# jianzongwu/betrayed-by-captions

Measured on AMD Instinct MI355X. Metric: images/sec (COCO-shaped 1024x1024, 100 queries, forward-only), higher is better.
Workload: dtype f32; 1 GPU; configs[1]: R50 + 100 queries, 1024x1024, batch 2/GPU, forward-only; global_batch=2, parallelism=replicas x1, precision=fp32 (parity mode, f16x3 MFMA), hip_graph=True, x3_overflow=False, library_fallbacks=0

## Files before the change

betrayed-by-captions_amd/_lib.py:

```python
import ctypes
import os

import torch

_HERE = os.path.dirname(os.path.abspath(__file__))
LIB_PATH = os.path.join(_HERE, 'lib', 'libcgg_hip.so')

CGG_F32 = 0
CGG_BF16 = 1

_c_int = ctypes.c_int
_c_vp = ctypes.c_void_p
_c_f = ctypes.c_float
_c_i64 = ctypes.c_int64

PROTOTYPES = {
    'cgg_version': (_c_int, []),
    'cgg_init': (_c_int, [_c_int]),
    'cgg_msda_forward_fused_vld': (_c_int, [_c_vp, _c_int, _c_vp, _c_vp, _c_vp, _c_int, _c_vp, _c_vp] + [_c_int] * 7 + [_c_vp]),
    'cgg_msda_backward_hostlevels_ws': (_c_int, [_c_vp, _c_int] + [_c_vp] * 8 + [_c_int] * 8 + [_c_vp, _c_i64, _c_vp, _c_vp]),
    'cgg_msda_backward_workspace_bytes': (_c_i64, [_c_vp, _c_vp] + [_c_int] * 7),
    'cgg_msda_read_levels': (_c_int, [_c_vp, _c_vp, _c_int, _c_int, _c_vp, _c_vp, _c_vp]),
    'cgg_last_error_string': (ctypes.c_char_p, []),
    'cgg_msda_forward': (_c_int, [_c_vp] * 6 + [_c_int] * 8 + [_c_vp]),
# ... 61 lines not shown
                       [_c_int] * 4 + [_c_vp]),
    'cgg_conv_x3_nhwc': (_c_int, [_c_vp] * 5 + [_c_int] * 10 + [_c_vp]),
    'cgg_gemm_x3s': (_c_int, [_c_vp, _c_int, _c_vp, _c_vp, _c_vp, _c_int, _c_int, _c_int, _c_vp, _c_int, _c_int] + [_c_int] * 4 + [_c_vp]),
    'cgg_gemm_x3s_batched': (_c_int, [_c_vp, _c_int, _c_int, _c_i64, _c_vp, _c_vp, _c_vp, _c_int, _c_int, _c_int, _c_vp, _c_int, _c_int] + [_c_int] * 4 + [_c_vp]),
    'cgg_conv_x3s_nhwc': (_c_int, [_c_vp] * 4 + [_c_int, _c_vp, _c_int] + [_c_int] * 10 + [_c_vp]),
    'cgg_x3a_encode': (_c_int, [_c_vp, _c_vp, _c_i64, _c_vp]),
    'cgg_x3a_decode': (_c_int, [_c_vp, _c_vp, _c_i64, _c_vp]),
    'cgg_x3_overflow_check': (_c_int, [_c_int, _c_vp, _c_vp]),
    'cgg_gemm_x3s_cfg': (_c_int, [_c_vp, _c_int, _c_vp, _c_vp, _c_vp, _c_int, _c_int, _c_int, _c_vp, _c_int, _c_int] + [_c_int] * 5 + [_c_vp]),
    'cgg_conv_x3s_nhwc_cfg': (_c_int, [_c_vp] * 4 + [_c_int, _c_vp, _c_int] + [_c_int] * 11 + [_c_vp]),
    'cgg_bias_relu_maxpool_nhwc_f32_x3a': (_c_int, [_c_vp] * 3 + [_c_int] * 4 + [_c_vp]),
    'cgg_group_norm_nhwc_f32_x3a': (_c_int, [_c_vp] * 4 + [_c_int] * 4 + [_c_f, _c_int, _c_vp, _c_int, _c_int, _c_i64, _c_int, _c_vp,
                                             _c_i64, _c_vp, _c_vp, _c_vp]),
    'cgg_encoder_layer_tail_x3a': (_c_int, [_c_vp] * 6 + [_c_f] + [_c_vp] * 6 + [_c_f, _c_vp, _c_int, _c_vp, _c_vp] +
                                   [_c_int] * 3 + [_c_vp]),
    'cgg_wgrad_x3_workspace_bytes': (_c_i64, [_c_int] * 3),
    'cgg_wgrad_x3': (_c_int, [_c_vp, _c_int, _c_vp, _c_int, _c_vp, _c_vp] + [_c_int] * 3 + [_c_vp]),
    'cgg_wgrad_bias_x3': (_c_int, [_c_vp, _c_int, _c_vp, _c_int, _c_vp, _c_vp, _c_vp] + [_c_int] * 3 + [_c_vp]),
    'cgg_transpose_f32': (_c_int, [_c_vp, _c_vp, _c_int, _c_int, _c_int, _c_vp]),
    'cgg_nchw_to_nhwc_pad1_f32': (_c_int, [_c_vp, _c_vp] + [_c_int] * 4 + [_c_vp]),
    'cgg_topk_select': (_c_int, [_c_vp, _c_int, _c_int, _c_int, _c_int, _c_vp, _c_vp]),
    'cgg_absmax_f32': (_c_int, [_c_vp, _c_int, _c_int, _c_int, _c_vp, _c_vp]),
    'cgg_relu_bwd_absmax_f32': (_c_int, [_c_vp, _c_vp, _c_vp, ctypes.c_longlong, _c_vp, _c_vp]),
    'cgg_gemm_x3_bwd': (_c_int, [_c_vp, _c_int, _c_vp, _c_vp, _c_vp, _c_int, _c_vp, _c_int, _c_vp] + [_c_int] * 3 + [_c_vp]),
    'cgg_gemm_x3_scaled': (_c_int, [_c_vp, _c_int, _c_vp, _c_vp, _c_vp, _c_vp, _c_int, _c_vp, _c_int] + [_c_int] * 4 + [_c_vp]),
    'cgg_conv_x3_nhwc_scaled': (_c_int, [_c_vp] * 6 + [_c_int] * 10 + [_c_vp]),
    'cgg_wgrad_x3_scaled': (_c_int, [_c_vp, _c_int, _c_vp, _c_vp, _c_int, _c_vp, _c_vp, _c_vp] + [_c_int] * 3 + [_c_vp]),
    'cgg_layernorm_chain': (_c_int, [_c_vp, _c_int, _c_vp, _c_vp, _c_f, _c_vp, _c_int, _c_vp, _c_vp, _c_f, _c_vp, _c_vp,
                                     _c_vp, _c_int, _c_int, _c_int, _c_i64, _c_vp]),
    'cgg_msda_prologue': (_c_int, [_c_vp, _c_int, _c_vp, _c_vp, _c_vp, _c_vp] + [_c_int] * 5 + [_c_vp]),
# ... 115 lines not shown
```

betrayed-by-captions_amd/csrc/norm.hip:

```cpp
#include "x3.h"

#define GN_CHUNK 16384

template <int VEC>
__global__ __launch_bounds__(256) void cgg_gn_partial_kernel(const float* __restrict__ x,
                                                             float* __restrict__ part, long long row_len,
                                                             int chunks) {
  const int row = blockIdx.y, chunk = blockIdx.x;
  const long long beg = (long long)chunk * GN_CHUNK;
  const long long end = min(row_len, beg + GN_CHUNK);
  const float* xr = x + (size_t)row * row_len;
  float s = 0.f, ss = 0.f;
  if (VEC == 4) {
    for (long long i = beg + threadIdx.x * 4; i < end; i += 256 * 4) {
      const f32x4 v = *reinterpret_cast<const f32x4*>(xr + i);
      s += (v[0] + v[1]) + (v[2] + v[3]);
      ss += (v[0] * v[0] + v[1] * v[1]) + (v[2] * v[2] + v[3] * v[3]);
    }
  } else {
    for (long long i = beg + threadIdx.x; i < end; i += 256) {
      const float v = xr[i];
      s += v;
      ss += v * v;
    }
// ... 366 lines not shown
                                              int W, float* y_padded, cgg_stream_t stream) {
  CGG_REQUIRE(y_padded && W > 0 && HW % W == 0, CGG_EINVAL, "cgg_group_norm_nhwc_f32_padout: null output / bad W");
  return gnh_launch(true, x, gamma, beta, ws, B, HW, C, groups, eps, relu, up_src, up_h, up_w, up_bstride, W, y_padded,
                    (int64_t)(HW / W + 2) * (W + 2) * C, nullptr, nullptr, nullptr, 0, stream, nullptr, 0, W);
}

extern "C" int cgg_group_norm_nhwc_f32_x3a(const float* x, const float* gamma, const float* beta, void* ws, int B, int HW, int C,
                                           int groups, float eps, int relu, const void* up_src_x3a, int up_h, int up_w,
                                           int64_t up_bstride, int W, void* y_x3a, int64_t y_bstride, const float* pos,
                                           void* yp_x3a, cgg_stream_t stream) {
  CGG_REQUIRE(y_x3a, CGG_EINVAL, "cgg_group_norm_nhwc_f32_x3a: null output");
  return gnh_launch(true, x, gamma, beta, ws, B, HW, C, groups, eps, relu, (const float*)up_src_x3a, up_h, up_w, up_bstride, W,
                    (float*)y_x3a, y_bstride, nullptr, pos, nullptr, 0, stream, (float*)yp_x3a, up_src_x3a ? 3 : 1);
}

template <bool RELU>
__global__ __launch_bounds__(256) void cgg_gn_nhwc_bwd_partials_kernel(const float* __restrict__ x, const float* __restrict__ y,
                                                                      const float* __restrict__ dy, const float* __restrict__ stats,
                                                                      float eps, float* __restrict__ part, int HW, int G, int ppb) {
  __shared__ float red[16][256];
  const int b = blockIdx.y, tid = threadIdx.x;
  const int g = tid % G, pl = tid / G, PL = 256 / G;
  const int p0 = blockIdx.x * ppb, p1 = min(p0 + ppb, HW);
  const float mean = stats[((size_t)b * G + g) * 2], rstd = rsqrtf(stats[((size_t)b * G + g) * 2 + 1] + eps);
  float dg[8], db[8];
#pragma unroll
  for (int k = 0; k < 8; ++k) dg[k] = db[k] = 0.f;
  for (int p = p0 + pl; p < p1; p += PL) {
    const size_t o = (((size_t)b * HW + p) * G + g) * 8;
    const f32x4 xa = *reinterpret_cast<const f32x4*>(x + o), xb = *reinterpret_cast<const f32x4*>(x + o + 4);
// ... 183 lines not shown
```

betrayed-by-captions_amd/mask2former_head.py:

```python
import copy
import os
import json
import warnings

import torch
import torch.distributed as dist
import torch.nn as nn
import torch.nn.functional as F

from . import ops, runtime
from .assigner import get_uncertain_point_coords_with_randomness, point_sample
from .bert_embeddings import BertEmbeddings
from .config import ConfigDict, to_config_dict
from .registry import (HEADS, build_assigner, build_head, build_loss, build_plugin_layer,
                       build_positional_encoding, build_sampler, build_transformer_layer_sequence)

POINT_LOGITS_X3 = os.environ.get('CGG_POINT_LOGITS_X3', '1') != '0'
BOS_TOKEN = 101
EOS_TOKEN = 102


def get_dist_info():
    if dist.is_available() and dist.is_initialized():
        return dist.get_rank(), dist.get_world_size()
# ... 486 lines not shown

    @staticmethod
    def _pack_stream(mf, sizes):
        H4, W4 = int(mf.shape[1]), int(mf.shape[2])
        pools = []
        for (h, w) in sizes:
            s = H4 // h
            pools.append(s if (h * s == H4 and w * s == W4 and s in (2, 4, 8)) else None)
        uniq = [1] + sorted({p for p in pools if p is not None})
        if len(uniq) <= 4:
            packed = dict(zip(uniq, ops.pack_mask_feature_nhwc_multi(mf, uniq)))
        else:
            packed = {p: ops.pack_mask_feature_nhwc(mf, p) for p in uniq}
        return packed[1], [packed[p] if p is not None else None for p in pools]

    def _finish_encode(self, enc):
        if enc.get('x3a'):
            sizes, memorys = enc['sizes'], enc['memorys']
            mf = enc['mf'] if 'mf' in enc else self.pixel_decoder.stream_fpn_x3a(*enc['fpn'])
            H4, W4 = int(mf.shape[1]), int(mf.shape[2])
            pools = []
            for h, w in sizes:
                s = H4 // h
                pools.append(s if (h * s == H4 and w * s == W4 and s in (2, 4, 8)) else None)
            uniq = [1] + sorted({p for p in pools if p is not None})
            packed = dict(zip(uniq, ops.pack_mask_feature_nhwc_x3(mf, uniq)))
            return dict(stream=True, kvs=self._project_kv_x3a(memorys, sizes), sizes=sizes, packed_full=packed[1],
                        pooled=[packed[p] if p is not None else None for p in pools], mask_features=None)
        kv16, sizes = enc['kv16'], enc['sizes']
        mf = enc['mf'] if 'mf' in enc else self.pixel_decoder.stream_fpn(*enc['fpn'])
        L = self.num_transformer_feat_level
        layers = self.transformer_decoder.layers
        H4, W4 = int(mf.shape[1]), int(mf.shape[2])
        packed_full, pooled = self._pack_stream(mf, sizes)
        kvs = self._project_kv_levels(kv16)
        return dict(stream=True, kvs=kvs, sizes=sizes, packed_full=packed_full, pooled=pooled, mask_features=None)

    def _project_kv_levels(self, kv16):
        L = self.num_transformer_feat_level
        layers = self.transformer_decoder.layers
        nl = self.num_transformer_decoder_layers
# ... 62 lines not shown
                return dict(stream=True, deferred=True, mf=mf, kv16=kv16, sizes=[level_hw[i] for i in range(L)])
            for i in range(L):
                sizes.append(level_hw[i])
                if kv16 is None:
                    mems.append(memorys[i] + self.level_embed.weight[i].view(1, 1, -1))
                    poss.append(self.decoder_positional_encoding.flat_unpadded(level_hw[i][0], level_hw[i][1], mf.device))
            packed_full, pooled = self._pack_stream(mf, sizes)
        elif (hasattr(pd, 'stream_ready_x3') and pd.stream_ready_x3(feats) and pd.num_outs >= L
              and all(isinstance(p, nn.Identity) for p in self.decoder_input_projs)
              and self.transformer_decoder.post_norm is not None and self.query_embed.weight.shape[1] % 32 == 0
              and all(l.stream_ready() for l in self.transformer_decoder.layers)):
            if defer_tail and runtime.x3a_enabled():
                mf, memorys, level_hw = pd.forward_stream_x3(feats, defer_fpn=defer_tail == 2)
                return dict(stream=True, deferred=True, x3a=True, memorys=memorys, sizes=[level_hw[i] for i in range(L)],
                            **({'fpn': mf} if defer_tail == 2 else {'mf': mf}))
            mf, memorys, level_hw = pd.forward_stream_x3(feats)
            mask_features = None
            H4, W4 = int(mf.shape[1]), int(mf.shape[2])
            pools = []
            x3a_mem = all(ops.is_x3a(m) for m in memorys[:L])
            for i in range(L):
                h, w = level_hw[i]
                sizes.append((h, w))
                if not x3a_mem:
                    mems.append(memorys[i] + self.level_embed.weight[i].view(1, 1, -1))
                    poss.append(self.decoder_positional_encoding.flat_unpadded(h, w, mf.device))
                s = H4 // h
                pools.append(s if (h * s == H4 and w * s == W4 and s in (2, 4, 8)) else None)
            uniq = [1] + sorted({p for p in pools if p is not None})
            packed = dict(zip(uniq, ops.pack_mask_feature_nhwc_x3(mf, uniq)))
            packed_full, pooled = packed[1], [packed[p] if p is not None else None for p in pools]
            if x3a_mem:
                kvs = self._project_kv_x3a(memorys, sizes)
                return dict(stream=True, kvs=kvs, sizes=sizes, packed_full=packed_full, pooled=pooled, mask_features=None)
        else:
            if runtime.x3_enabled() and not torch.is_grad_enabled() and feats[0].is_cuda:
                runtime.note_fallback('pixel decoder / head', 'stream_ready_x3() is false for this configuration: module path on f32 '
                                      'library GEMMs')
            feats = [ops.x3a_to_f32(f) if ops.is_x3a(f) else f for f in feats]
            feats = [f.float().contiguous() if f.dtype != torch.float32 else f for f in feats]
            mask_features, memorys = pd(feats)
            mask_features = mask_features.contiguous()
            split = not runtime.is_bf16()
            H4, W4 = mask_features.shape[-2:]
            for i in range(L):
# ... 711 lines not shown
```

betrayed-by-captions_amd/ops.py:

```python
import ctypes
import os
import math

import torch

from . import _lib
from ._lib import CGG_BF16, CGG_F32, CggError, check, dev_ptr, stream_ptr

_WS_CACHE = {}

KERNEL_EVENTS = None


KERNEL_META = None


class _timed:
    def __init__(self, name, **meta):
        self.name = name
        self.meta = meta
        self.on = KERNEL_EVENTS is not None and not torch.cuda.is_current_stream_capturing()

    def __enter__(self):
        if self.on:
# ... 1130 lines not shown
    if x.dtype != torch.float32:
        raise CggError(f'group_norm_nhwc_x3a: x dtype {x.dtype}')
    need = _lib_().cgg_group_norm_nhwc_workspace_bytes(B, HW, int(groups))
    if ws is None or ws.numel() * ws.element_size() < need:
        raise CggError(f'group_norm_nhwc_x3a: workspace too small ({need} bytes needed; see group_norm_nhwc_workspace)')
    rc = _lib_().cgg_group_norm_nhwc_f32_x3a(
        dev_ptr(x, 'x', torch.float32), dev_ptr(gamma, 'gamma', torch.float32), dev_ptr(beta, 'beta', torch.float32),
        dev_ptr(ws, 'ws', torch.float32), B, HW, C, int(groups), float(eps), int(bool(relu)),
        _ptr_at(up[0], up[1]) if up is not None else None, up[3] if up is not None else 0,
        up[4] if up is not None else 0, up[2] if up is not None else 0, int(W),
        _ptr_at(out[0], out[1]), out[2], _ptr_at(pos[0], pos[1]) if pos is not None else None,
        _ptr_at(outp[0], outp[1]) if outp is not None else None, stream_ptr(x.device))
    check(rc, 'cgg_group_norm_nhwc_f32_x3a')


def zero_border_map(B, H, W, C, device):
    y = torch.empty((B, H + 2, W + 2, C), dtype=torch.float32, device=device)
    y[:, 0].zero_()
    y[:, H + 1].zero_()
    y[:, 1:H + 1, 0].zero_()
    y[:, 1:H + 1, W + 1].zero_()
    return y


def group_norm_nhwc_padout(x, gamma, beta, groups, eps, ws, hw, y_padded, relu=False, lo=None, lo_hw=None):
    B, HW, C = x.shape
    H, W = int(hw[0]), int(hw[1])
    if x.dtype != torch.float32 or not x.is_contiguous() or tuple(y_padded.shape) != (B, H + 2, W + 2, C) or not y_padded.is_contiguous():
        raise CggError('group_norm_nhwc_padout: x (B, HW, C) float32 contiguous and y_padded (B, H + 2, W + 2, C) expected')
    if lo is not None and (not lo.is_contiguous() or lo.dtype != torch.float32):
# ... 68 lines not shown
    for pool in pools:
        if H % pool or W % pool:
            raise CggError(f'pack_mask_feature_nhwc_x3: {H}x{W} not divisible by pool={pool}')
        h, w = H // pool, W // pool
        hi = torch.empty((B, (h * w + 31) // 32, C // 8, 32, 8), dtype=torch.bfloat16, device=feat.device)
        lo = torch.empty_like(hi)
        outs.append(PackedFeature(hi, lo, B, C, h, w))
        hp.append(hi.data_ptr())
        lp.append(lo.data_ptr())
    n = len(pools)
    rc = _lib_().cgg_pack_mask_feature_nhwc_f32_x3(dev_ptr(feat, 'mask_feature', torch.float32), (ctypes.c_void_p * n)(*hp),
                                                   (ctypes.c_void_p * n)(*lp), _int_array([int(p) for p in pools]), n,
                                                   B, C, H, W, stream_ptr(feat.device))
    check(rc, 'cgg_pack_mask_feature_nhwc_f32_x3')
    return outs


def pack_mask_feature_nhwc_multi(feat, pools):
    B, H, W, C = feat.shape
    outs, ptrs = [], []
    for pool in pools:
        if H % pool or W % pool:
            raise CggError(f'pack_mask_feature_nhwc: {H}x{W} not divisible by pool={pool}')
        h, w = H // pool, W // pool
        hi = torch.empty((B, (h * w + 31) // 32, C // 8, 32, 8), dtype=torch.bfloat16, device=feat.device)
        outs.append(PackedFeature(hi, None, B, C, h, w))
        ptrs.append(hi.data_ptr())
    n = len(pools)
    rc = _lib_().cgg_pack_mask_feature_nhwc_multi(dev_ptr(feat, 'mask_feature', torch.bfloat16),
                                                  (ctypes.c_void_p * n)(*ptrs), _int_array([int(p) for p in pools]), n,
# ... 905 lines not shown
```

betrayed-by-captions_amd/pixel_decoder.py:

```python
import math
import os

import torch
import torch.nn as nn
import torch.nn.functional as F

from . import ops, runtime
from .registry import (ATTENTION, FEEDFORWARD_NETWORK, PLUGIN_LAYERS, POSITIONAL_ENCODING,
                       TRANSFORMER_LAYER, TRANSFORMER_LAYER_SEQUENCE, build_attention,
                       build_feedforward_network, build_positional_encoding,
                       build_transformer_layer, build_transformer_layer_sequence)

FUSED_TAIL = os.environ.get('CGG_FUSED_TAIL', '1') != '0'
FUSED_TRAIN_MSDA = os.environ.get('CGG_FUSED_TRAIN_MSDA', '1') != '0'
FUSED_TRAIN_LN = os.environ.get('CGG_FUSED_TRAIN_LN', '1') != '0'
MERGED_PROJ = os.environ.get('CGG_MERGED_PROJ', '1') != '0' and not os.environ.get('CGG_MSDA_GENERIC')


def build_norm(cfg, num_features):
    cfg = dict(cfg)
    t = cfg.pop('type')
    requires_grad = cfg.pop('requires_grad', True)
    if t == 'GN':
        m = nn.GroupNorm(cfg.pop('num_groups'), num_features, **cfg)
# ... 792 lines not shown
        cache[key] = (ver, t)
        while len(cache) > 2 * len(self.encoder.layers):
            cache.popitem(last=False)
        return runtime.keepalive(t)

    @staticmethod
    def _merged_proj_ok(layer):
        attn = layer.attentions[0]
        so, aw, vp = attn.sampling_offsets, attn.attention_weights, attn.value_proj
        C, H = vp.weight.shape[1], attn.num_heads
        n_cat = so.weight.shape[0] + aw.weight.shape[0]
        return (MERGED_PROJ and H == 8 and C == 256 and vp.weight.shape[0] == 256 and attn.num_levels == 3 and attn.num_points == 4
                and n_cat == 3 * H * attn.num_levels * attn.num_points and (C + n_cat) % 32 == 0
                and all(m.bias is not None for m in (vp, so, aw)))

    def _forward_stream_x3a(self, feats, defer_fpn=False):
        B = feats[0].shape[0]
        dev = feats[0].device
        C = 256
        rows = lambda f: (f if ops.is_x3a(f) else ops.x3a_encode(ops.nchw_to_nhwc(f).contiguous()).permute(0, 3, 1, 2)) \
            .as_subclass(torch.Tensor).permute(0, 2, 3, 1).reshape(-1, f.shape[1])
        level_hw, level_start, N, pos, ref = self._stream_levels(feats)
        src = torch.empty((B, N, C), dtype=torch.float32, device=dev)
        need_srcp = not all(self._merged_proj_ok(l) for l in self.encoder.layers)
        srcp = torch.empty((B, N, C), dtype=torch.float32, device=dev) if need_srcp else None
        ws = ops.group_norm_nhwc_workspace(B, int(feats[0].shape[2]) * int(feats[0].shape[3]), 32, dev)
        for i in range(self.num_encoder_levels):
            f = feats[self.num_input_levels - i - 1]
            h, w = level_hw[i]
            cm = self.input_convs[i]
            y = runtime.linear_x3s(rows(f), cm.conv.weight.flatten(1), cm.conv.bias)
            gn = getattr(cm, cm.norm_name)
            ops.group_norm_nhwc_x3a(y.view(B, h * w, C), gn.weight, gn.bias, 32, gn.eps, ws, out=(src, level_start[i] * C, N * C),
                                    pos=(pos, level_start[i] * C) if need_srcp else None,
                                    outp=(srcp, level_start[i] * C) if need_srcp else None)
        src = self._encoder_stream_x3a(src, srcp, pos, ref, level_hw, level_start)
        mems = [ops.as_x3a(src[:, s0:s0 + h * w, :]) for s0, (h, w) in zip(level_start, level_hw)]
        fpn = (rows(feats[0]), int(feats[0].shape[2]), int(feats[0].shape[3]), src, level_start[-1], N, level_hw[-1], ws)
        if defer_fpn:
            return fpn, mems, level_hw
        return self.stream_fpn_x3a(*fpn), mems, level_hw

    def stream_fpn_x3a(self, frows, H4, W4, src, fine_start, N, fine_hw, ws):
        C = 256
        B = src.shape[0]
        lat, outc = self.lateral_convs[0], self.output_convs[0]
        hl, wl = fine_hw
        level_start = [fine_start]
        y = runtime.linear_x3s(frows, lat.conv.weight.flatten(1), lat.conv.bias).view(B, H4 * W4, C)
        gn = getattr(lat, lat.norm_name)
        ops.group_norm_nhwc_x3a(y, gn.weight, gn.bias, 32, gn.eps, ws, out=(y, 0, H4 * W4 * C),
                                up=(src, level_start[-1] * C, N * C, hl, wl), W=W4)
        w3 = runtime.derived_cached('x3_conv_image', (outc.conv.weight,), lambda: ops.pack_conv_weight_x3(outc.conv.weight))
        z = ops.conv_x3s_nhwc(y.view(B, H4, W4, C), w3, C, 3, 1, 1, outc.conv.bias, out_split=False).view(B, H4 * W4, C)
        gn = getattr(outc, outc.norm_name)
        ops.group_norm_nhwc_x3a(z, gn.weight, gn.bias, 32, gn.eps, ws, out=(z, 0, H4 * W4 * C), relu=True)
        mf = runtime.linear_x3s(z.view(B * H4 * W4, C), self.mask_feature.weight.flatten(1), self.mask_feature.bias)
        return mf.view(B, H4, W4, -1)

    def forward_stream_x3(self, feats, defer_fpn=False):
        if runtime.x3a_enabled():
            return self._forward_stream_x3a(feats, defer_fpn=defer_fpn)
        feats = [ops.x3a_to_f32(f) if ops.is_x3a(f) else f for f in feats]
        B = feats[0].shape[0]
        dev = feats[0].device
        C = 256
        level_hw, level_start, N, pos, ref = self._stream_levels(feats)
        src = torch.empty((B, N, C), dtype=torch.float32, device=dev)
        ws = ops.group_norm_nhwc_workspace(B, int(feats[0].shape[2]) * int(feats[0].shape[3]), 32, dev)
        for i in range(self.num_encoder_levels):
            f = feats[self.num_input_levels - i - 1]
            h, w = level_hw[i]
            cm = self.input_convs[i]
            y = runtime.linear_x3(ops.nchw_to_nhwc(f).reshape(B * h * w, f.shape[1]), cm.conv.weight.flatten(1), cm.conv.bias)
            gn = getattr(cm, cm.norm_name)
            ops.group_norm_nhwc(y.view(B, h * w, C), gn.weight, gn.bias, 32, gn.eps, ws, out32=(src, level_start[i] * C, N * C))
        src = self._encoder_stream_x3(src, pos, ref, level_hw, level_start)
# ... 103 lines not shown
```

include/cgg_hip.h:

```cpp
#ifndef CGG_HIP_H_
#define CGG_HIP_H_

#include <stdint.h>

#ifdef __cplusplus
extern "C" {
#endif

#define CGG_VERSION 100

#define CGG_OK 0
#define CGG_EINVAL (-1)
#define CGG_EUNSUPPORTED (-2)
#define CGG_EALIGN (-3)
#define CGG_ELIBRARY (-4)

#define CGG_F32 0
#define CGG_BF16 1
#define CGG_F32_BF16MFMA 2
#define CGG_F32_X3 3

typedef void* cgg_stream_t;

int cgg_version(void);
// ... 222 lines not shown
int cgg_group_norm_nhwc_f32_x3a(const float* x, const float* gamma, const float* beta, void* ws, int B, int HW, int C, int groups,
                                float eps, int relu, const void* up_src_x3a, int up_h, int up_w, int64_t up_bstride, int W,
                                void* y_x3a, int64_t y_bstride, const float* pos, void* yp_x3a, cgg_stream_t stream);

int64_t cgg_group_norm_nhwc_backward_workspace_bytes(int B, int HW, int groups);
int cgg_group_norm_nhwc_f32_backward(const float* x, const float* y, const float* dy, const float* stats, const float* gamma, void* ws,
                                     int B, int HW, int C, int groups, float eps, int relu, float* dx, float* tot, float* dlo, int lo_h,
                                     int lo_w, int W, int dx_padded, cgg_stream_t stream);
int cgg_group_norm_nhwc_f32_padout(const float* x, const float* gamma, const float* beta, void* ws, int B, int HW, int C, int groups,
                                   float eps, int relu, const float* up_src, int up_h, int up_w, int64_t up_bstride, int W,
                                   float* y_padded, cgg_stream_t stream);
int cgg_encoder_layer_tail_x3a(const float* a32, const void* x_x3a, const void* wo_x3, const float* bo, const float* gamma0,
                               const float* beta0, float eps0, const void* w1_x3, const float* b1, const void* w2_x3,
                               const float* b2, const float* gamma1, const float* beta1, float eps1, const float* pos,
                               int pos_rows, void* y_x3a, void* yp_x3a, int M, int C, int F, cgg_stream_t stream);

int cgg_transpose_f32(const float* in, float* out, int B, int R, int C, cgg_stream_t stream);
int cgg_nchw_to_nhwc_pad1_f32(const float* in, float* out, int B, int C, int H, int W, cgg_stream_t stream);

int64_t cgg_wgrad_x3_workspace_bytes(int M, int N, int K);
int cgg_wgrad_x3(const float* dy, int ldy, const float* x, int ldx, float* ws, int* splits_out, int M, int N, int K,
                 cgg_stream_t stream);
int cgg_wgrad_bias_x3(const float* dy, int ldy, const float* x, int ldx, float* ws, float* ws_bias, int* splits_out, int M, int N,
                      int K, cgg_stream_t stream);

int cgg_topk_select(const float* x, int ld, int rows, int N, int k, int64_t* idx, cgg_stream_t stream);

int cgg_absmax_f32(const float* x, int ld, int M, int N, float* amax, cgg_stream_t stream);
int cgg_relu_bwd_absmax_f32(const float* gy, const float* y, float* g, long long n, float* amax, cgg_stream_t stream);
int cgg_gemm_x3_bwd(const float* a, int lda, const float* a_amax, const void* w_x3, const float* mask, int ldm, float* out, int ldc,
// ... 125 lines not shown
```

Before: 385.2 images/sec.

## Fuse GroupNorm apply, mask-feature linear, and multi-scale x3 packing into one kernel

Adds a fused kernel for the mask-feature head that normalizes the FPN output with precomputed GroupNorm stats, applies ReLU, runs the 256x256 mask_feature projection with split-f16 MFMA, and writes the pooled x3-packed images for every requested scale in one pass. A separate stats-only GroupNorm entry point supplies mean and variance beforehand. This removes the full normalized-activation write/read, the separate GEMM launch and the separate pack pass, at the cost of a large LDS tile per block. It is only used when the caller passes pack_pools and the shape checks pass; otherwise the old three-step path runs.

```diff
diff --git a/betrayed-by-captions_amd/_lib.py b/betrayed-by-captions_amd/_lib.py
--- a/betrayed-by-captions_amd/_lib.py
+++ b/betrayed-by-captions_amd/_lib.py
@@ -99,6 +99,9 @@
                                              _c_i64, _c_vp, _c_vp, _c_vp]),
     'cgg_encoder_layer_tail_x3a': (_c_int, [_c_vp] * 6 + [_c_f] + [_c_vp] * 6 + [_c_f, _c_vp, _c_int, _c_vp, _c_vp] +
                                    [_c_int] * 3 + [_c_vp]),
+    'cgg_group_norm_nhwc_f32_stats': (_c_int, [_c_vp, _c_vp] + [_c_int] * 4 + [_c_vp]),
+    'cgg_mask_feature_head_x3': (_c_int, [_c_vp] * 4 + [_c_f, _c_int] + [_c_vp] * 5 + [_c_int, _c_vp] + [_c_int] * 5 + [_c_vp]),
+    'cgg_mask_feature_head_x3_cfg': (_c_int, [_c_vp] * 4 + [_c_f, _c_int] + [_c_vp] * 5 + [_c_int, _c_vp] + [_c_int] * 6 + [_c_vp]),
     'cgg_wgrad_x3_workspace_bytes': (_c_i64, [_c_int] * 3),
     'cgg_wgrad_x3': (_c_int, [_c_vp, _c_int, _c_vp, _c_int, _c_vp, _c_vp] + [_c_int] * 3 + [_c_vp]),
     'cgg_wgrad_bias_x3': (_c_int, [_c_vp, _c_int, _c_vp, _c_int, _c_vp, _c_vp, _c_vp] + [_c_int] * 3 + [_c_vp]),
diff --git a/betrayed-by-captions_amd/csrc/mask_feature_head.hip b/betrayed-by-captions_amd/csrc/mask_feature_head.hip
--- /dev/null
+++ b/betrayed-by-captions_amd/csrc/mask_feature_head.hip
@@ -0,0 +1,304 @@
+#include "x3.h"
+
+typedef __attribute__((ext_vector_type(4))) uint32_t mh_u32x4;
+
+#define MH_C 256
+#define MH_STEPS 16
+#define MH_RB 64
+#define MH_TS 260
+#define MH_IMG (2 * MH_STEPS * 64)
+
+struct MhJobs {
+  int n;
+  int pool[4], Wp[4], npix[4], T[4];
+  mh_u32x4* hi[4];
+  mh_u32x4* lo[4];
+};
+
+template <int NWV>
+__global__ __launch_bounds__(64 * NWV, NWV / 2) void cgg_mask_feature_head_x3_kernel(
+    const float* __restrict__ z, const float* __restrict__ ws, const float* __restrict__ gamma, const float* __restrict__ beta,
+    float eps, const CggX3W w, const float* __restrict__ bias, float lo_clamp, const MhJobs jobs, float* __restrict__ mf, int H, int W,
+    int* __restrict__ flag) {
+  extern __shared__ __attribute__((aligned(16))) unsigned char mh_smem[];
+  mh_u32x4* xfrag = reinterpret_cast<mh_u32x4*>(mh_smem);
+  float* tile = reinterpret_cast<float*>(mh_smem);
+  constexpr int NT = 64 * NWV;
+  constexpr int TN = 8 / NWV;
+  constexpr int MH_PF = NWV == 8 ? 2 : 4;
+  const int tid = threadIdx.x, lane = tid & 63, wn = tid >> 6;
+  const int j = lane & 31, hi5 = lane >> 5;
+  const int b = blockIdx.y;
+  const int tiles_x = W >> 3;
+  const int by = blockIdx.x / tiles_x, bx = blockIdx.x - by * tiles_x;
+  const int y0 = by * 8, x0 = bx * 8;
+  const size_t HW = (size_t)H * W;
+
+  mh_u32x4 qh[TN][MH_PF], ql[TN][MH_PF];
+  const mh_u32x4 *bh[TN], *bl[TN];
+#pragma unroll
+  for (int t = 0; t < TN; ++t) {
+    const size_t o = ((size_t)(TN * wn + t) * MH_STEPS) * 64 + lane;
+    bh[t] = w.hi + o;
+    bl[t] = w.lo + o;
+#pragma unroll
+    for (int s = 0; s < MH_PF; ++s) {
+      qh[t][s] = bh[t][s * 64];
+      ql[t][s] = bl[t][s * 64];
+    }
+  }
+  float am = 0.f;
+  {
+    constexpr int NP = MH_RB * 32 / NT;
+    const int k8 = tid & 31;
+    f32x4 v0[NP], v1[NP];
+#pragma unroll
+    for (int i = 0; i < NP; ++i) {
+      const int row = (tid + i * NT) >> 5;
+      const size_t pix = (size_t)(y0 + (row >> 3)) * W + x0 + (row & 7);
+      const float* src = z + ((size_t)b * HW + pix) * MH_C + 8 * k8;
+      v0[i] = *reinterpret_cast<const f32x4*>(src);
+      v1[i] = *reinterpret_cast<const f32x4*>(src + 4);
+    }
+    const float mean = ws[((size_t)b * 32 + k8) * 2], var = ws[((size_t)b * 32 + k8) * 2 + 1];
+    const f32x4 ga = *reinterpret_cast<const f32x4*>(gamma + k8 * 8), gb = *reinterpret_cast<const f32x4*>(gamma + k8 * 8 + 4);
+    const f32x4 ba = *reinterpret_cast<const f32x4*>(beta + k8 * 8), bb = *reinterpret_cast<const f32x4*>(beta + k8 * 8 + 4);
+    __builtin_amdgcn_sched_barrier(0);
+    const float rstd = rsqrtf(var + eps);
+#pragma unroll
+    for (int i = 0; i < NP; ++i) {
+      const int row = (tid + i * NT) >> 5;
+      float f[8];
+#pragma unroll
+      for (int k = 0; k < 4; ++k) {
+        f[k] = (v0[i][k] - mean) * rstd * ga[k] + ba[k];
+        f[k + 4] = (v1[i][k] - mean) * rstd * gb[k] + bb[k];
+      }
+#pragma unroll
+      for (int k = 0; k < 8; ++k) {
+        f[k] = fmaxf(f[k], 0.f);
+        am = fmaxf(am, fabsf(f[k]));
+      }
+      mh_u32x4 h, l;
+      cgg_x3_split8(f32x4{f[0], f[1], f[2], f[3]}, f32x4{f[4], f[5], f[6], f[7]}, h, l);
+      const int slot = ((row >> 5) * MH_STEPS + (k8 >> 1)) * 64 + (((row & 31) + 32 * (k8 & 1)) ^ (k8 >> 1));
+      xfrag[slot] = h;
+      xfrag[MH_IMG + slot] = l;
+    }
+  }
+  if (flag && !(am * CGG_X3_ASCALE <= CGG_X3A_MAX)) atomicOr(flag, 1);
+  f32x16 acc[2][TN];
+#pragma unroll
+  for (int a = 0; a < 2; ++a)
+#pragma unroll
+    for (int t = 0; t < TN; ++t)
+#pragma unroll
+      for (int r = 0; r < 16; ++r) acc[a][t][r] = 0.f;
+  __syncthreads();
+  {
+    int xl = lane;
+    asm volatile("" : "+v"(xl));
+    auto load_a = [&](int s, mh_u32x4& h0, mh_u32x4& l0, mh_u32x4& h1, mh_u32x4& l1) {
+      const int xo = xl ^ s;
+      h0 = xfrag[s * 64 + xo];
+      l0 = xfrag[MH_IMG + s * 64 + xo];
+      h1 = xfrag[(MH_STEPS + s) * 64 + xo];
+      l1 = xfrag[MH_IMG + (MH_STEPS + s) * 64 + xo];
+    };
+    mh_u32x4 ah0, al0, ah1, al1;
+    load_a(0, ah0, al0, ah1, al1);
+#pragma unroll
+    for (int s = 0; s < MH_STEPS; ++s) {
+      mh_u32x4 bhv[TN], blv[TN];
+#pragma unroll
+      for (int t = 0; t < TN; ++t) {
+        bhv[t] = qh[t][s % MH_PF];
+        blv[t] = ql[t][s % MH_PF];
+      }
+      const mh_u32x4 vah0 = ah0, val0 = al0, vah1 = ah1, val1 = al1;
+      if (s + 1 < MH_STEPS) load_a(s + 1, ah0, al0, ah1, al1);
+      if (s + MH_PF < MH_STEPS) {
+#pragma unroll
+        for (int t = 0; t < TN; ++t) {
+          qh[t][s % MH_PF] = bh[t][(s + MH_PF) * 64];
+          ql[t][s % MH_PF] = bl[t][(s + MH_PF) * 64];
+        }
+      }
+      __builtin_amdgcn_sched_barrier(0);
+#define MH_MF(A, B, C) C = __builtin_amdgcn_mfma_f32_32x32x16_f16(__builtin_bit_cast(f16x8, A), __builtin_bit_cast(f16x8, B), C, 0, 0, 0)
+#pragma unroll
+      for (int t = 0; t < TN; ++t) {
+        MH_MF(val0, bhv[t], acc[0][t]);
+        MH_MF(val1, bhv[t], acc[1][t]);
+      }
+#pragma unroll
+      for (int t = 0; t < TN; ++t) {
+        MH_MF(vah0, blv[t], acc[0][t]);
+        MH_MF(vah1, blv[t], acc[1][t]);
+      }
+#pragma unroll
+      for (int t = 0; t < TN; ++t) {
+        MH_MF(vah0, bhv[t], acc[0][t]);
+        MH_MF(vah1, bhv[t], acc[1][t]);
+      }
+#undef MH_MF
+      __builtin_amdgcn_sched_barrier(0);
+    }
+  }
+  __syncthreads();
+#pragma unroll
+  for (int nt = 0; nt < TN; ++nt) {
+    const int col = 32 * TN * wn + 32 * nt + j;
+    const float cs = w.scale[col] * CGG_X3_ASCALE;
+    const float bs = bias ? bias[col] * CGG_X3_ASCALE : 0.f;
+#pragma unroll
+    for (int mt = 0; mt < 2; ++mt)
+#pragma unroll
+      for (int r = 0; r < 16; ++r) {
+        const float v = fmaxf(acc[mt][nt][r] * cs + bs, lo_clamp);
+        tile[(32 * mt + (r & 3) + 8 * (r >> 2) + 4 * hi5) * MH_TS + col] = v * CGG_X3_INV_ASCALE;
+      }
+  }
+  __syncthreads();
+  for (int jb = 0; jb < jobs.n; ++jb) {
+    const int pool = jobs.pool[jb], Wp = jobs.Wp[jb], T = jobs.T[jb];
+    mh_u32x4* __restrict__ dh = jobs.hi[jb];
+    mh_u32x4* __restrict__ dl = jobs.lo[jb];
+    if (pool == 1) {
+#pragma unroll
+      for (int it = 0; it < MH_RB * 32 / NT; ++it) {
+        const int idx = tid + it * NT;
+        const int tx = idx & 7, kc = (idx >> 3) & 31, ty = idx >> 8;
+        const float* s = tile + (ty * 8 + tx) * MH_TS + kc * 8;
+        const f32x4 v0 = *reinterpret_cast<const f32x4*>(s), v1 = *reinterpret_cast<const f32x4*>(s + 4);
+        mh_u32x4 h, l;
+        cgg_x3_split8(v0, v1, h, l);
+        const int p = (y0 + ty) * W + x0 + tx;
+        const size_t slot = (((size_t)b * T + (p >> 5)) * 32 + kc) * 32 + (p & 31);
+        dh[slot] = h;
+        dl[slot] = l;
+      }
+    } else {
+      const int ns = 8 / pool, npp = ns * ns;
+      for (int idx = tid; idx < npp * 32; idx += NT) {
+        const int pp = idx & (npp - 1), kc = idx / npp;
+        const int ii = pp / ns, jj = pp - ii * ns;
+        const int r0 = pool * ii + (pool >> 1) - 1, c0 = pool * jj + (pool >> 1) - 1;
+        const float* s00 = tile + (r0 * 8 + c0) * MH_TS + kc * 8;
+        const float* s10 = s00 + 8 * MH_TS;
+        f32x4 m[2];
+#pragma unroll
+        for (int h = 0; h < 2; ++h) {
+          const f32x4 a = *reinterpret_cast<const f32x4*>(s00 + 4 * h), c = *reinterpret_cast<const f32x4*>(s00 + MH_TS + 4 * h);
+          const f32x4 d = *reinterpret_cast<const f32x4*>(s10 + 4 * h), e = *reinterpret_cast<const f32x4*>(s10 + MH_TS + 4 * h);
+          m[h] = ((a + c) + (d + e)) * 0.25f;
+        }
+        mh_u32x4 h, l;
+        cgg_x3_split8(m[0], m[1], h, l);
+        const int p = (y0 / pool + ii) * Wp + x0 / pool + jj;
+        const size_t slot = (((size_t)b * T + (p >> 5)) * 32 + kc) * 32 + (p & 31);
+        dh[slot] = h;
+        dl[slot] = l;
+      }
+    }
+    const int rag = jobs.npix[jb] & 31;
+    if (rag && blockIdx.x == gridDim.x - 1) {
+      const int cnt = 32 - rag;
+      const mh_u32x4 zero = {0u, 0u, 0u, 0u};
+      for (int idx = tid; idx < cnt * 32; idx += NT) {
+        const int kc = idx / cnt, pl = rag + (idx - kc * cnt);
+        const size_t slot = (((size_t)b * T + (T - 1)) * 32 + kc) * 32 + pl;
+        dh[slot] = zero;
+        dl[slot] = zero;
+      }
+    }
+  }
+  if (mf) {
+#pragma unroll
+    for (int it = 0; it < MH_RB * 32 / NT; ++it) {
+      const int idx = tid + it * NT;
+      const int row = idx >> 5, c8 = idx & 31;
+      const float* s = tile + row * MH_TS + c8 * 8;
+      const size_t pix = (size_t)(y0 + (row >> 3)) * W + x0 + (row & 7);
+      float* o = mf + ((size_t)b * HW + pix) * MH_C + c8 * 8;
+      *reinterpret_cast<f32x4*>(o) = *reinterpret_cast<const f32x4*>(s);
+      *reinterpret_cast<f32x4*>(o + 4) = *reinterpret_cast<const f32x4*>(s + 4);
+    }
+  }
+}
+
+int* cgg_x3_overflow_flag_ptr();
+
+constexpr int MH_DEFAULT_CFG = 1;
+
+template <int NWV>
+static int mh_go(const char* who, const float* z, const void* gn_ws, const float* gamma, const float* beta, float eps, const void* w_x3,
+                 const float* bias, const MhJobs& jobs, float* mf, int B, int H, int W, hipStream_t stream) {
+  constexpr size_t lds = (size_t)MH_RB * MH_TS * sizeof(float);
+  static_assert(lds >= (size_t)2 * MH_IMG * 16, "the tile must cover the row images");
+  static bool attr_set[16] = {false};
+  int dev = 0;
+  (void)hipGetDevice(&dev);
+  if (dev < 0 || dev >= 16 || !attr_set[dev]) {
+    hipError_t e = hipFuncSetAttribute((const void*)cgg_mask_feature_head_x3_kernel<NWV>, hipFuncAttributeMaxDynamicSharedMemorySize, (int)lds);
+    CGG_REQUIRE(e == hipSuccess, (int)e, "%s: cannot raise dynamic LDS to %zu", who, lds);
+    if (dev >= 0 && dev < 16) attr_set[dev] = true;
+  }
+  hipLaunchKernelGGL(cgg_mask_feature_head_x3_kernel<NWV>, dim3((unsigned)((H / 8) * (W / 8)), (unsigned)B), dim3(64 * NWV), lds, stream, z,
+                     (const float*)gn_ws, gamma, beta, eps, cgg_x3_view(w_x3, MH_C, MH_C), bias, -__builtin_inff(), jobs, mf, H, W,
+                     cgg_x3_overflow_flag_ptr());
+  CGG_CHECK_LAUNCH(who);
+  return CGG_OK;
+}
+
+static int mh_launch(const char* who, const float* z, const void* gn_ws, const float* gamma, const float* beta, float eps, int groups,
+                     const void* w_x3, const float* bias, void* const* hi_host, void* const* lo_host, const int* pools_host, int n,
+                     float* mf, int B, int H, int W, int C, int N, int cfg, cgg_stream_t stream) {
+  CGG_REQUIRE(z && gn_ws && gamma && beta && w_x3 && hi_host && lo_host && pools_host, CGG_EINVAL, "%s: null pointer", who);
+  CGG_REQUIRE(B > 0 && B <= 65535 && H > 0 && W > 0 && n >= 1 && n <= 4, CGG_EINVAL, "%s: bad sizes", who);
+  CGG_REQUIRE(C == MH_C && N == MH_C && groups == 32, CGG_EUNSUPPORTED, "%s: C=%d N=%d groups=%d (only 256 / 256 / 32 is built)", who, C,
+              N, groups);
+  CGG_REQUIRE(H % 8 == 0 && W % 8 == 0, CGG_EUNSUPPORTED, "%s: %dx%d must be multiples of the 8 x 8 tile", who, H, W);
+  CGG_REQUIRE((long long)H * W < (1ll << 31), CGG_EUNSUPPORTED, "%s: map too large", who);
+  CGG_REQUIRE(cfg >= -1 && cfg <= 1, CGG_EINVAL, "%s: configuration %d (0, 1, or -1 = default)", who, cfg);
+  CGG_REQUIRE(cgg_aligned16(z) && cgg_aligned16(gamma) && cgg_aligned16(beta) && cgg_aligned16(w_x3) && cgg_aligned16(mf) &&
+                  (((uintptr_t)gn_ws) & 3u) == 0 && (((uintptr_t)bias) & 3u) == 0,
+              CGG_EALIGN, "%s: 16-B alignment", who);
+  MhJobs jobs;
+  jobs.n = n;
+  for (int i = 0; i < 4; ++i) {
+    jobs.pool[i] = jobs.Wp[i] = jobs.npix[i] = jobs.T[i] = 0;
+    jobs.hi[i] = jobs.lo[i] = nullptr;
+  }
+  for (int i = 0; i < n; ++i) {
+    const int pool = pools_host[i];
+    CGG_REQUIRE(pool == 1 || pool == 2 || pool == 4 || pool == 8, CGG_EUNSUPPORTED, "%s: pool=%d must be 1, 2, 4 or 8", who, pool);
+    CGG_REQUIRE(hi_host[i] && lo_host[i] && cgg_aligned16(hi_host[i]) && cgg_aligned16(lo_host[i]), CGG_EALIGN, "%s: output %d", who, i);
+    const int Hp = H / pool, Wp = W / pool;
+    jobs.pool[i] = pool;
+    jobs.Wp[i] = Wp;
+    jobs.npix[i] = Hp * Wp;
+    jobs.T[i] = (Hp * Wp + 31) / 32;
+    jobs.hi[i] = (mh_u32x4*)hi_host[i];
+    jobs.lo[i] = (mh_u32x4*)lo_host[i];
+  }
+  if ((cfg < 0 ? MH_DEFAULT_CFG : cfg) == 0)
+    return mh_go<4>(who, z, gn_ws, gamma, beta, eps, w_x3, bias, jobs, mf, B, H, W, (hipStream_t)stream);
+  return mh_go<8>(who, z, gn_ws, gamma, beta, eps, w_x3, bias, jobs, mf, B, H, W, (hipStream_t)stream);
+}
+
+extern "C" int cgg_mask_feature_head_x3(const float* z, const void* gn_ws, const float* gamma, const float* beta, float eps, int groups,
+                                        const void* w_x3, const float* bias, void* const* hi_host, void* const* lo_host,
+                                        const int* pools_host, int n, float* mf, int B, int H, int W, int C, int N,
+                                        cgg_stream_t stream) {
+  return mh_launch("cgg_mask_feature_head_x3", z, gn_ws, gamma, beta, eps, groups, w_x3, bias, hi_host, lo_host, pools_host, n, mf, B, H,
+                   W, C, N, -1, stream);
+}
+
+extern "C" int cgg_mask_feature_head_x3_cfg(const float* z, const void* gn_ws, const float* gamma, const float* beta, float eps,
+                                            int groups, const void* w_x3, const float* bias, void* const* hi_host, void* const* lo_host,
+                                            const int* pools_host, int n, float* mf, int B, int H, int W, int C, int N, int cfg,
+                                            cgg_stream_t stream) {
+  return mh_launch("cgg_mask_feature_head_x3_cfg", z, gn_ws, gamma, beta, eps, groups, w_x3, bias, hi_host, lo_host, pools_host, n, mf,
+                   B, H, W, C, N, cfg, stream);
+}
diff --git a/betrayed-by-captions_amd/csrc/norm.hip b/betrayed-by-captions_amd/csrc/norm.hip
--- a/betrayed-by-captions_amd/csrc/norm.hip
+++ b/betrayed-by-captions_amd/csrc/norm.hip
@@ -404,6 +404,23 @@
                     (float*)y_x3a, y_bstride, nullptr, pos, nullptr, 0, stream, (float*)yp_x3a, up_src_x3a ? 3 : 1);
 }
 
+extern "C" int cgg_group_norm_nhwc_f32_stats(const float* x, void* ws, int B, int HW, int C, int groups, cgg_stream_t stream) {
+  CGG_REQUIRE(x && ws, CGG_EINVAL, "cgg_group_norm_nhwc_f32_stats: null pointer");
+  CGG_REQUIRE(B > 0 && HW > 0 && C > 0 && groups > 0, CGG_EINVAL, "cgg_group_norm_nhwc_f32_stats: bad sizes");
+  CGG_REQUIRE(C == groups * 8 && groups <= 256 && 256 % groups == 0, CGG_EUNSUPPORTED,
+              "cgg_group_norm_nhwc_f32_stats: needs C / groups == 8 and groups | 256 (C=%d, groups=%d)", C, groups);
+  CGG_REQUIRE(cgg_aligned16(x) && (((uintptr_t)ws) & 7u) == 0, CGG_EALIGN, "cgg_group_norm_nhwc_f32_stats: alignment");
+  hipStream_t s = (hipStream_t)stream;
+  const int nblk = (HW + GNH_PIX - 1) / GNH_PIX;
+  const int head = B * groups * 2;
+  hipLaunchKernelGGL(cgg_gn_nhwc_stats_kernel<true>, dim3(nblk, B), dim3(256), 0, s, (const uint4*)x, (float*)ws, HW, groups, GNH_PIX,
+                     head);
+  const float inv_n = 1.f / ((float)HW * 8.f);
+  hipLaunchKernelGGL(cgg_gn_nhwc_reduce_kernel, dim3(B * groups), dim3(64), 0, s, (float*)ws, head, nblk, groups, B, x, HW, inv_n);
+  CGG_CHECK_LAUNCH("cgg_group_norm_nhwc_f32_stats");
+  return CGG_OK;
+}
+
 template <bool RELU>
 __global__ __launch_bounds__(256) void cgg_gn_nhwc_bwd_partials_kernel(const float* __restrict__ x, const float* __restrict__ y,
                                                                       const float* __restrict__ dy, const float* __restrict__ stats,
diff --git a/betrayed-by-captions_amd/mask2former_head.py b/betrayed-by-captions_amd/mask2former_head.py
--- a/betrayed-by-captions_amd/mask2former_head.py
+++ b/betrayed-by-captions_amd/mask2former_head.py
@@ -524,17 +524,25 @@
             packed = {p: ops.pack_mask_feature_nhwc(mf, p) for p in uniq}
         return packed[1], [packed[p] if p is not None else None for p in pools]
 
+    @staticmethod
+    def _x3_pools(H4, W4, sizes):
+        pools = []
+        for h, w in sizes:
+            s = H4 // h
+            pools.append(s if (h * s == H4 and w * s == W4 and s in (2, 4, 8)) else None)
+        return pools, [1] + sorted({p for p in pools if p is not None})
+
     def _finish_encode(self, enc):
         if enc.get('x3a'):
             sizes, memorys = enc['sizes'], enc['memorys']
-            mf = enc['mf'] if 'mf' in enc else self.pixel_decoder.stream_fpn_x3a(*enc['fpn'])
-            H4, W4 = int(mf.shape[1]), int(mf.shape[2])
-            pools = []
-            for h, w in sizes:
-                s = H4 // h
-                pools.append(s if (h * s == H4 and w * s == W4 and s in (2, 4, 8)) else None)
-            uniq = [1] + sorted({p for p in pools if p is not None})
-            packed = dict(zip(uniq, ops.pack_mask_feature_nhwc_x3(mf, uniq)))
+            if 'mf' in enc:
+                mf = enc['mf']
+                pools, uniq = self._x3_pools(int(mf.shape[1]), int(mf.shape[2]), sizes)
+            else:
+                fpn = enc['fpn']
+                pools, uniq = self._x3_pools(int(fpn[1]), int(fpn[2]), sizes)
+                mf = self.pixel_decoder.stream_fpn_x3a(*fpn[:8], pack_pools=uniq)
+            packed = mf if isinstance(mf, dict) else dict(zip(uniq, ops.pack_mask_feature_nhwc_x3(mf, uniq)))
             return dict(stream=True, kvs=self._project_kv_x3a(memorys, sizes), sizes=sizes, packed_full=packed[1],
                         pooled=[packed[p] if p is not None else None for p in pools], mask_features=None)
         kv16, sizes = enc['kv16'], enc['sizes']
@@ -627,21 +635,20 @@
                 mf, memorys, level_hw = pd.forward_stream_x3(feats, defer_fpn=defer_tail == 2)
                 return dict(stream=True, deferred=True, x3a=True, memorys=memorys, sizes=[level_hw[i] for i in range(L)],
                             **({'fpn': mf} if defer_tail == 2 else {'mf': mf}))
-            mf, memorys, level_hw = pd.forward_stream_x3(feats)
+            fl = list(feats)
+            H4, W4 = int(fl[0].shape[2]), int(fl[0].shape[3])
+            pools, uniq = self._x3_pools(H4, W4, [(int(f.shape[2]), int(f.shape[3]))
+                                                  for f in (fl[pd.num_input_levels - i - 1] for i in range(L))])
+            mf, memorys, level_hw = pd.forward_stream_x3(feats, pack_pools=uniq)
             mask_features = None
-            H4, W4 = int(mf.shape[1]), int(mf.shape[2])
-            pools = []
             x3a_mem = all(ops.is_x3a(m) for m in memorys[:L])
             for i in range(L):
                 h, w = level_hw[i]
                 sizes.append((h, w))
                 if not x3a_mem:
                     mems.append(memorys[i] + self.level_embed.weight[i].view(1, 1, -1))
-                    poss.append(self.decoder_positional_encoding.flat_unpadded(h, w, mf.device))
-                s = H4 // h
-                pools.append(s if (h * s == H4 and w * s == W4 and s in (2, 4, 8)) else None)
-            uniq = [1] + sorted({p for p in pools if p is not None})
-            packed = dict(zip(uniq, ops.pack_mask_feature_nhwc_x3(mf, uniq)))
+                    poss.append(self.decoder_positional_encoding.flat_unpadded(h, w, fl[0].device))
+            packed = mf if isinstance(mf, dict) else dict(zip(uniq, ops.pack_mask_feature_nhwc_x3(mf, uniq)))
             packed_full, pooled = packed[1], [packed[p] if p is not None else None for p in pools]
             if x3a_mem:
                 kvs = self._project_kv_x3a(memorys, sizes)
diff --git a/betrayed-by-captions_amd/ops.py b/betrayed-by-captions_amd/ops.py
--- a/betrayed-by-captions_amd/ops.py
+++ b/betrayed-by-captions_amd/ops.py
@@ -1168,6 +1168,17 @@
     check(rc, 'cgg_group_norm_nhwc_f32_x3a')
 
 
+def group_norm_nhwc_stats(x, groups, ws):
+    if x.dim() != 3 or x.dtype != torch.float32 or not x.is_contiguous():
+        raise CggError('group_norm_nhwc_stats: x must be a contiguous (B, HW, C) float32 tensor')
+    B, HW, C = x.shape
+    need = _lib_().cgg_group_norm_nhwc_workspace_bytes(B, HW, int(groups))
+    if ws is None or ws.dtype != torch.float32 or ws.numel() * ws.element_size() < need:
+        raise CggError(f'group_norm_nhwc_stats: workspace too small ({need} bytes needed; see group_norm_nhwc_workspace)')
+    check(_lib_().cgg_group_norm_nhwc_f32_stats(dev_ptr(x, 'x', torch.float32), dev_ptr(ws, 'ws', torch.float32), B, HW, C, int(groups),
+                                                stream_ptr(x.device)), 'cgg_group_norm_nhwc_f32_stats')
+
+
 def zero_border_map(B, H, W, C, device):
     y = torch.empty((B, H + 2, W + 2, C), dtype=torch.float32, device=device)
     y[:, 0].zero_()
@@ -1266,6 +1277,76 @@
                                                    B, C, H, W, stream_ptr(feat.device))
     check(rc, 'cgg_pack_mask_feature_nhwc_f32_x3')
     return outs
+
+
+_MFH_C = 256
+_MFH_W_BYTES = 2 * (_MFH_C // 32) * (_MFH_C // 16) * 64 * 16 + (_MFH_C // 32) * 32 * 4
+
+
+def _mfh_problem(z, ws, gn, weight_x3, bias, pools):
+    def f32_dev(t, n=None):
+        return (torch.is_tensor(t) and t.dtype == torch.float32 and t.is_cuda and t.is_contiguous() and t.data_ptr() % 16 == 0
+                and (n is None or t.numel() == n))
+    if not (torch.is_tensor(z) and z.dim() == 4 and f32_dev(z)):
+        return 'z must be a contiguous, 16-byte aligned (B, H, W, C) float32 ROCm tensor'
+    B, H, W, C = (int(s) for s in z.shape)
+    if C != _MFH_C or B < 1 or B > 65535:
+        return f'C={C} (only {_MFH_C} is built) / B={B}'
+    if H < 8 or W < 8 or H % 8 or W % 8:
+        return f'{H}x{W} is not a multiple of the 8 x 8 tile'
+    if not (isinstance(gn, (tuple, list)) and len(gn) == 4):
+        return 'gn must be (gamma, beta, eps, groups)'
+    gamma, beta, _, groups = gn
+    if int(groups) != 32 or not f32_dev(gamma, C) or not f32_dev(beta, C):
+        return 'GroupNorm must have 32 groups and contiguous float32 ROCm gamma / beta of 256'
+    if not (f32_dev(ws) and ws.numel() >= B * 32 * 2):
+        return 'ws must be the float32 GroupNorm workspace (>= B * 32 * 2 floats)'
+    if not (is_x3(weight_x3) and weight_x3.is_cuda and weight_x3.is_contiguous() and weight_x3.data_ptr() % 16 == 0
+            and weight_x3.numel() * weight_x3.element_size() == _MFH_W_BYTES):
+        return 'weight_x3 must be the x3 image of a (256, 256) weight'
+    if bias is not None and not f32_dev(bias, _MFH_C):
+        return 'bias must be a contiguous float32 ROCm tensor of 256'
+    pools = list(pools) if pools is not None else []
+    if not 1 <= len(pools) <= 4 or any(p not in (1, 2, 4, 8) or H % p or W % p for p in pools) or len(set(pools)) != len(pools):
+        return f'pools={pools}: 1 to 4 distinct values out of 1, 2, 4, 8 that divide {H}x{W}'
+    devs = {t.device for t in (z, ws, gamma, beta, weight_x3) + ((bias,) if bias is not None else ())}
+    if len(devs) != 1:
+        return 'operands on different devices'
+    return None
+
+
+def mask_feature_head_x3_ok(z, ws, gn, weight_x3, bias, pools, want_f32=False):
+    try:
+        return _mfh_problem(z, ws, gn, weight_x3, bias, pools) is None
+    except Exception:
+        return False
+
+
+def mask_feature_head_x3(z, ws, gn, weight_x3, bias, pools, want_f32=False, cfg=-1):
+    why = _mfh_problem(z, ws, gn, weight_x3, bias, pools)
+    if why is not None:
+        raise CggError(f'mask_feature_head_x3: {why}')
+    B, H, W, C = (int(s) for s in z.shape)
+    gamma, beta, eps, groups = gn
+    pools = [int(p) for p in pools]
+    outs, hp, lp = {}, [], []
+    for pool in pools:
+        h, w = H // pool, W // pool
+        hi = torch.empty((B, (h * w + 31) // 32, C // 8, 32, 8), dtype=torch.bfloat16, device=z.device)
+        lo = torch.empty_like(hi)
+        outs[pool] = PackedFeature(hi, lo, B, C, h, w)
+        hp.append(hi.data_ptr())
+        lp.append(lo.data_ptr())
+    mf = torch.empty((B, H, W, C), dtype=torch.float32, device=z.device) if want_f32 else None
+    n = len(pools)
+    with _timed('mask_feature_head_x3', flops=2.0 * B * H * W * C * C, bytes=4.0 * B * H * W * C * (2.4 + (1 if want_f32 else 0)),
+                shape=(B * H * W, C, C)):
+        rc = _lib_().cgg_mask_feature_head_x3_cfg(
+            dev_ptr(z), dev_ptr(ws), dev_ptr(gamma), dev_ptr(beta), float(eps), int(groups), dev_ptr(weight_x3),
+            dev_ptr(bias) if bias is not None else None, (ctypes.c_void_p * n)(*hp), (ctypes.c_void_p * n)(*lp), _int_array(pools), n,
+            dev_ptr(mf) if mf is not None else None, B, H, W, C, C, int(cfg), stream_ptr(z.device))
+    check(rc, 'cgg_mask_feature_head_x3')
+    return (outs, mf) if want_f32 else outs
 
 
 def pack_mask_feature_nhwc_multi(feat, pools):
diff --git a/betrayed-by-captions_amd/pixel_decoder.py b/betrayed-by-captions_amd/pixel_decoder.py
--- a/betrayed-by-captions_amd/pixel_decoder.py
+++ b/betrayed-by-captions_amd/pixel_decoder.py
@@ -830,7 +830,7 @@
                 and n_cat == 3 * H * attn.num_levels * attn.num_points and (C + n_cat) % 32 == 0
                 and all(m.bias is not None for m in (vp, so, aw)))
 
-    def _forward_stream_x3a(self, feats, defer_fpn=False):
+    def _forward_stream_x3a(self, feats, defer_fpn=False, pack_pools=None):
         B = feats[0].shape[0]
         dev = feats[0].device
         C = 256
@@ -852,12 +852,12 @@
                                     outp=(srcp, level_start[i] * C) if need_srcp else None)
         src = self._encoder_stream_x3a(src, srcp, pos, ref, level_hw, level_start)
         mems = [ops.as_x3a(src[:, s0:s0 + h * w, :]) for s0, (h, w) in zip(level_start, level_hw)]
-        fpn = (rows(feats[0]), int(feats[0].shape[2]), int(feats[0].shape[3]), src, level_start[-1], N, level_hw[-1], ws)
+        fpn = (rows(feats[0]), int(feats[0].shape[2]), int(feats[0].shape[3]), src, level_start[-1], N, level_hw[-1], ws, pack_pools)
         if defer_fpn:
             return fpn, mems, level_hw
         return self.stream_fpn_x3a(*fpn), mems, level_hw
 
-    def stream_fpn_x3a(self, frows, H4, W4, src, fine_start, N, fine_hw, ws):
+    def stream_fpn_x3a(self, frows, H4, W4, src, fine_start, N, fine_hw, ws, pack_pools=None):
         C = 256
         B = src.shape[0]
         lat, outc = self.lateral_convs[0], self.output_convs[0]
@@ -870,13 +870,21 @@
         w3 = runtime.derived_cached('x3_conv_image', (outc.conv.weight,), lambda: ops.pack_conv_weight_x3(outc.conv.weight))
         z = ops.conv_x3s_nhwc(y.view(B, H4, W4, C), w3, C, 3, 1, 1, outc.conv.bias, out_split=False).view(B, H4 * W4, C)
         gn = getattr(outc, outc.norm_name)
+        if pack_pools is not None:
+            wm = self.mask_feature.weight.flatten(1)
+            bm = self.mask_feature.bias.detach() if self.mask_feature.bias is not None else None
+            wk = runtime.derived_cached('x3_image', (wm,), lambda: ops.pack_linear_weight_x3(wm))
+            head = (z.view(B, H4, W4, C), ws, (gn.weight, gn.bias, gn.eps, gn.num_groups), wk, bm, list(pack_pools))
+            if ops.mask_feature_head_x3_ok(*head):
+                ops.group_norm_nhwc_stats(z, 32, ws)
+                return ops.mask_feature_head_x3(*head)
         ops.group_norm_nhwc_x3a(z, gn.weight, gn.bias, 32, gn.eps, ws, out=(z, 0, H4 * W4 * C), relu=True)
         mf = runtime.linear_x3s(z.view(B * H4 * W4, C), self.mask_feature.weight.flatten(1), self.mask_feature.bias)
         return mf.view(B, H4, W4, -1)
 
-    def forward_stream_x3(self, feats, defer_fpn=False):
+    def forward_stream_x3(self, feats, defer_fpn=False, pack_pools=None):
         if runtime.x3a_enabled():
-            return self._forward_stream_x3a(feats, defer_fpn=defer_fpn)
+            return self._forward_stream_x3a(feats, defer_fpn=defer_fpn, pack_pools=pack_pools)
         feats = [ops.x3a_to_f32(f) if ops.is_x3a(f) else f for f in feats]
         B = feats[0].shape[0]
         dev = feats[0].device
diff --git a/include/cgg_hip.h b/include/cgg_hip.h
--- a/include/cgg_hip.h
+++ b/include/cgg_hip.h
@@ -260,6 +260,14 @@
                                const float* beta0, float eps0, const void* w1_x3, const float* b1, const void* w2_x3,
                                const float* b2, const float* gamma1, const float* beta1, float eps1, const float* pos,
                                int pos_rows, void* y_x3a, void* yp_x3a, int M, int C, int F, cgg_stream_t stream);
+int cgg_group_norm_nhwc_f32_stats(const float* x, void* ws, int B, int HW, int C, int groups, cgg_stream_t stream);
+int cgg_mask_feature_head_x3(const float* z, const void* gn_ws, const float* gamma, const float* beta, float eps, int groups,
+                             const void* w_x3, const float* bias, void* const* hi_host, void* const* lo_host, const int* pools_host,
+                             int n, float* mf, int B, int H, int W, int C, int N, cgg_stream_t stream);
+int cgg_mask_feature_head_x3_cfg(const float* z, const void* gn_ws, const float* gamma, const float* beta, float eps, int groups,
+                                 const void* w_x3, const float* bias, void* const* hi_host, void* const* lo_host,
+                                 const int* pools_host, int n, float* mf, int B, int H, int W, int C, int N, int cfg,
+                                 cgg_stream_t stream);
 
 int cgg_transpose_f32(const float* in, float* out, int B, int R, int C, cgg_stream_t stream);
 int cgg_nchw_to_nhwc_pad1_f32(const float* in, float* out, int B, int C, int H, int W, cgg_stream_t stream);
diff --git a/scratch/mask_feature_head_bench.py b/scratch/mask_feature_head_bench.py
--- /dev/null
+++ b/scratch/mask_feature_head_bench.py
@@ -0,0 +1,106 @@
+import os
+import sys
+
+sys.path.insert(0, os.path.dirname(os.path.dirname(os.path.abspath(__file__))))
+import torch
+import cgg_amd
+from cgg_amd import ops, runtime
+
+dev = torch.device('cuda')
+C, G, EPS, N_LAUNCH, ROUNDS, COPIES = 256, 32, 1e-5, 20, 5, 4
+POOLS = [1, 2, 4, 8]
+lines = []
+
+
+def say(s):
+    print(s, flush=True)
+    lines.append(s)
+
+
+def timeit(fn, n=N_LAUNCH):
+    torch.cuda.synchronize()
+    s, e = torch.cuda.Event(enable_timing=True), torch.cuda.Event(enable_timing=True)
+    s.record()
+    for i in range(n):
+        fn(i)
+    e.record()
+    torch.cuda.synchronize()
+    return s.elapsed_time(e) / n * 1e3
+
+
+def run(B, H, W):
+    g = torch.Generator().manual_seed(H)
+    r = lambda *s, k=1.0: (torch.randn(*s, generator=g) * k).to(dev)
+    zs = [r(B, H * W, C) for _ in range(COPIES)]
+    gamma, beta, wt, bias = 1 + 0.1 * r(C), 0.1 * r(C), r(C, C, k=1 / 16), 0.1 * r(C)
+    wk = ops.pack_linear_weight_x3(wt)
+    ws = ops.group_norm_nhwc_workspace(B, H * W, G, dev)
+    a = torch.empty_like(zs[0])
+    gn = (gamma, beta, EPS, G)
+
+    def stats(i):
+        ops.group_norm_nhwc_stats(zs[i % COPIES], G, ws)
+
+    def gn_full(i):
+        ops.group_norm_nhwc_x3a(zs[i % COPIES], gamma, beta, G, EPS, ws, out=(a, 0, H * W * C), relu=True)
+
+    def gemm(i):
+        return runtime.linear_x3s(a.view(B * H * W, C), wt, bias)
+
+    mf = gemm(0)
+
+    def pack(i):
+        return ops.pack_mask_feature_nhwc_x3(mf.view(B, H, W, C), POOLS)
+
+    def three(i):
+        gn_full(i)
+        return ops.pack_mask_feature_nhwc_x3(gemm(i).view(B, H, W, C), POOLS)
+
+    def fused_cfg(cfg):
+        def f(i):
+            z = zs[i % COPIES]
+            ops.group_norm_nhwc_stats(z, G, ws)
+            return ops.mask_feature_head_x3(z.view(B, H, W, C), ws, gn, wk, bias, POOLS, cfg=cfg)
+        return f
+
+    def head_only(cfg):
+        return lambda i: ops.mask_feature_head_x3(zs[i % COPIES].view(B, H, W, C), ws, gn, wk, bias, POOLS, cfg=cfg)
+
+    old = three(0)
+    new = fused_cfg(-1)(0)
+    same = all(torch.equal(new[p].hi.view(torch.int16), o.hi.view(torch.int16)) and
+               torch.equal(new[p].lo.view(torch.int16), o.lo.view(torch.int16)) for p, o in zip(POOLS, old))
+    fns = dict(three=three, fused_4w=fused_cfg(0), fused_8w=fused_cfg(1), stats=stats, gn_full=gn_full, gemm=gemm, pack=pack,
+               head_4w=head_only(0), head_8w=head_only(1))
+    for f in fns.values():
+        for i in range(3):
+            f(i)
+    t = {k: [] for k in fns}
+    for _ in range(ROUNDS):
+        for k, f in fns.items():
+            t[k].append(timeit(f))
+    med = {k: sorted(v)[len(v) // 2] for k, v in t.items()}
+    say(f'(B, H, W) = ({B}, {H}, {W}): {B * H * W} rows, pools {POOLS}; images bit-identical: {same}')
+    for k in fns:
+        say(f'  {k:9s} median {med[k]:7.1f} us   runs ' + ' '.join(f'{x:.1f}' for x in t[k]))
+    byts = B * H * W * C * 4 * (1 + 1 + sum(1.0 / (p * p) for p in POOLS[1:]))
+    for k in ('fused_4w', 'fused_8w'):
+        say(f'  {k} saves {med["three"] - med[k]:.1f} us = {100 * (1 - med[k] / med["three"]):.1f} % of the three-call sum '
+            f'(slowest fused run {max(t[k]):.1f} vs fastest three-call run {min(t["three"]):.1f})')
+    for k in ('head_4w', 'head_8w'):
+        say(f'  {k}: {byts / med[k] / 1e6:.2f} TB/s of the {byts / 1e6:.0f} MB it must move, '
+            f'{2.0 * 3 * B * H * W * C * C / med[k] / 1e6:.0f} TF/s f16')
+    rep = med['gn_full'] - med['stats'] + med['gemm'] + med['pack']
+    say(f'  apply pass = gn_full - stats = {med["gn_full"] - med["stats"]:.1f} us; the three replaced kernels, timed apart = {rep:.1f} us')
+    for k in ('head_4w', 'head_8w'):
+        say(f'  {k} alone vs the three replaced kernels: saves {rep - med[k]:.1f} us = {100 * (1 - med[k] / rep):.1f} %')
+    return same
+
+
+ok = True
+for shape in ((2, 256, 256), (2, 200, 336)):
+    ok = run(*shape) and ok
+if len(sys.argv) > 1:
+    with open(sys.argv[1], 'w') as f:
+        f.write('\n'.join(lines) + '\n')
+sys.exit(0 if ok else 1)
```

Result: faster. 391.7 images/sec, median of 6 (+1.7%).
